# ModelTC/Dipoorlet

Measured on AMD Instinct MI355X. Metric: calibration images/sec (whole node) + achieved HBM GB/s, ResNet-50 ONNX N=1024, -A hist, higher is better.
Workload: dtype f32; 1 GPU; ResNet-50 ONNX activation set (T=123, 26598376 fp32 elems/img), -A hist --bins 2048, N=1024 per GPU in 32 batches of 32: range pass + histogram pass + percentile clip; device=AMD Radeon Graphics (gfx950:sramecc+:xnack-), hist_checksum_ok=True, world_size_seen_by_backend=1

## Files before the change

dipoorlet_amd/csrc/calib_kernels.hip:

```cpp
#include "common.hpp"

#pragma clang fp contract(off)

namespace {

struct MinMaxOp {
    float mn, mx;
    uint32_t nan;
    __device__ __forceinline__ void operator()(float x) {
        mn = fminf(mn, x);
        mx = fmaxf(mx, x);
        nan |= (x != x);
    }
};

__device__ __forceinline__ void minmax_commit(const MinMaxOp& op, uint32_t slot, float* s_mn, float* s_mx, uint32_t* s_nan,
                                              uint32_t* __restrict__ min_enc, uint32_t* __restrict__ max_enc,
                                              uint32_t* __restrict__ nan_flag) {
    float mn = wave_min(op.mn), mx = wave_max(op.mx);
    uint32_t nn = __any(op.nan) ? 1u : 0u;
    const int w = threadIdx.x / kWave;
    if ((threadIdx.x & (kWave - 1)) == 0) {
        s_mn[w] = mn;
        s_mx[w] = mx;
        s_nan[w] = nn;
    }
    __syncthreads();
    if (threadIdx.x == 0) {
#pragma unroll
        for (int j = 1; j < kBlock / kWave; ++j) {
            mn = fminf(mn, s_mn[j]);
            mx = fmaxf(mx, s_mx[j]);
            nn |= s_nan[j];
        }
        if (mn <= mx) {
            atomicMin(min_enc + slot, enc_f32(mn));
            atomicMax(max_enc + slot, enc_f32(mx));
        }
        if (nn) atomicOr(nan_flag + slot, 1u);
    }
    __syncthreads();
}

__global__ __launch_bounds__(kBlock) void k_minmax(const dpl_work_item* __restrict__ items,
                                                    const uint32_t* __restrict__ bb,
                                                    const float* const* __restrict__ segs,
                                                    uint32_t* __restrict__ min_enc, uint32_t* __restrict__ max_enc,
                                                    uint32_t* __restrict__ nan_flag) {
    __shared__ float s_mn[kBlock / kWave], s_mx[kBlock / kWave];
    __shared__ uint32_t s_nan[kBlock / kWave];
    uint32_t k0, k1;
    block_items(bb, k0, k1);
    for (uint32_t k = k0; k < k1; ++k) {
        const dpl_work_item it = items[k];
        MinMaxOp op{INFINITY, -INFINITY, 0u};
        stream_span(segs[it.seg] + it.offset, it.count, op);
        minmax_commit(op, it.slot, s_mn, s_mx, s_nan, min_enc, max_enc, nan_flag);
    }
}

__global__ void k_minmax_init(uint32_t* mn, uint32_t* mx, uint32_t* nan, int64_t n) {
    int64_t i = (int64_t)blockIdx.x * blockDim.x + threadIdx.x;
    if (i < n) {
        mn[i] = 0xFFFFFFFFu;
        mx[i] = 0u;
        nan[i] = 0u;
    }
}

__device__ __forceinline__ void minmax_decode(uint32_t mn, uint32_t mx, uint32_t nan, float& omn, float& omx) {
    const bool bad = nan != 0u || mn == 0xFFFFFFFFu;
    omn = bad ? NAN : dec_f32(mn);
    omx = bad ? NAN : dec_f32(mx);
}

__global__ void k_minmax_finalize(const uint32_t* mn, const uint32_t* mx, const uint32_t* nan, int64_t n,
                                  float* omn, float* omx) {
    int64_t i = (int64_t)blockIdx.x * blockDim.x + threadIdx.x;
    if (i < n) minmax_decode(mn[i], mx[i], nan[i], omn[i], omx[i]);
}

__global__ void k_minmax_encode(const float* mn, const float* mx, int64_t n, uint32_t* emn, uint32_t* emx,
                                uint32_t* nan) {
    int64_t i = (int64_t)blockIdx.x * blockDim.x + threadIdx.x;
    if (i < n) {
        const bool bad = (mn[i] != mn[i]) || (mx[i] != mx[i]);
        emn[i] = bad ? 0xFFFFFFFFu : enc_f32(mn[i]);
        emx[i] = bad ? 0u : enc_f32(mx[i]);
        nan[i] = bad ? 1u : 0u;
    }
}

__device__ __forceinline__ float hist_edge(int i, float step, float first) {
    return __fadd_rn(__fmul_rn((float)i, step), first);
}

template <bool kFast>
struct HistOp {
    uint32_t* lds;
    float first, last, step, inv, denom;
    int last_bin;
    float fbins;
    uint32_t nonzero;
    __device__ __forceinline__ void operator()(float x) {
        const float a = fabsf(x);
        const bool nz = (a != 0.0f);
        nonzero += nz;
        if (kFast) {
            if (nz && (a <= last)) {
                const int i = (int)__fmul_rn(a, inv);
                const uint32_t dec = (a < __fmul_rn((float)i, step)) ? 0xFFFFFFFCu : 0u;
                atomicAdd(reinterpret_cast<uint32_t*>(reinterpret_cast<char*>(lds) + (((uint32_t)i << 2) + dec)), 1u);
            }
            return;
        }
        int i;
        if (kFast) {
            i = (int)__fmul_rn(a, inv);
            i = i > last_bin ? last_bin : i;
            i -= (a < __fmul_rn((float)i, step)) ? 1 : 0;
        } else {
            i = (int)__fmul_rn(__fdiv_rn(__fsub_rn(a, first), denom), fbins);
            i = i > last_bin ? last_bin : i;
            i = i < 0 ? 0 : i;
            i -= (a < hist_edge(i, step, first)) ? 1 : 0;
            i += (i != last_bin && a >= hist_edge(i + 1, step, first)) ? 1 : 0;
        }
        if (nz && (a <= last)) atomicAdd(lds + i, 1u);
    }
};

template <bool kFast>
__device__ __forceinline__ void hist_op_init(HistOp<kFast>& op, const dpl_hist_range& r, int bins, uint32_t* lds) {
    op.lds = lds;
    op.first = r.first;
    op.last = r.last;
    op.step = r.step;
    op.inv = r.inv;
    op.denom = __fsub_rn(r.last, r.first);
    op.last_bin = bins - 1;
    op.fbins = (float)bins;
    op.nonzero = 0u;
}

template <class Count>
__device__ __forceinline__ void hist_flush(uint32_t nonzero, const dpl_work_item& it, const dpl_hist_range& r, int bins,
                                           Count* __restrict__ hist, uint32_t* lds, uint32_t* s_nz) {
    const uint32_t nzw = wave_sum(nonzero);
    if ((threadIdx.x & (kWave - 1)) == 0) s_nz[threadIdx.x / kWave] = nzw;
    __syncthreads();
    if (threadIdx.x == 0) {
        uint32_t nzb = 0;
        for (int k = 0; k < kBlock / kWave; ++k) nzb += s_nz[k];
        const uint32_t z = it.count - nzb;
        if (z) atomicAdd(lds + r.zero_bin, z);
        const uint32_t top = lds[bins];
        if (top) atomicAdd(lds + bins - 1, top);
    }
    __syncthreads();
    Count* __restrict__ out = hist + (uint64_t)it.slot * (uint64_t)bins;
    for (int b = threadIdx.x; b < bins; b += kBlock) {
        const uint32_t c = lds[b];
        if (c) {
            if constexpr (sizeof(Count) == 8)
                atomicAdd(reinterpret_cast<unsigned long long*>(out + b), (unsigned long long)c);
            else
                atomicAdd(out + b, c);
        }
    }
}

template <bool kFast>
__device__ __forceinline__ void hist_body(const dpl_work_item& it, const float* const* __restrict__ segs,
                                          const dpl_hist_range& r, int bins, uint64_t* __restrict__ hist,
                                          uint32_t* lds, uint32_t* s_nz) {
    HistOp<kFast> op;
    hist_op_init(op, r, bins, lds);
    stream_span(segs[it.seg] + it.offset, it.count, op);
    hist_flush(op.nonzero, it, r, bins, hist, lds, s_nz);
}

__global__ __launch_bounds__(kBlock) void k_abs_hist(const dpl_work_item* __restrict__ items,
                                                      const uint32_t* __restrict__ bb,
                                                      const float* const* __restrict__ segs,
                                                      const dpl_hist_range* __restrict__ ranges, int bins,
                                                      uint64_t* __restrict__ hist) {
    extern __shared__ __attribute__((aligned(16))) uint32_t lds[];
    uint32_t* s_nz = lds + bins + 1;
    uint32_t k0, k1;
    block_items(bb, k0, k1);
    for (uint32_t k = k0; k < k1; ++k) {
        const dpl_work_item it = items[k];
        const dpl_hist_range r = ranges[it.slot];
        if (r.status != 0u) continue;
        for (int b = threadIdx.x; b <= bins; b += kBlock) lds[b] = 0u;
        __syncthreads();
        if (r.exact_div)
            hist_body<false>(it, segs, r, bins, hist, lds, s_nz);
        else
            hist_body<true>(it, segs, r, bins, hist, lds, s_nz);
        __syncthreads();
    }
}

__device__ __forceinline__ float py_max(float a, float b) { return (b > a) ? b : a; }
__device__ __forceinline__ float py_min(float a, float b) { return (b < a) ? b : a; }

__device__ __forceinline__ dpl_hist_range hist_range_of(float gmin, float gmax, int bins) {
    dpl_hist_range r;
    const float dmax = py_max(gmax, -gmin);
    float first = 0.0f, last = dmax;
    r.dmax = dmax;
    r.status = 0u;
    if (!(fabsf(last) <= 3.402823466e+38f) || last < first) r.status = 1u;
    if (first == last) {
        first = -0.5f;
        last = 0.5f;
    }
    const float delta = __fsub_rn(last, first);
    const float fb = (float)bins;
    r.first = first;
    r.last = last;
    r.step = __fdiv_rn(delta, fb);
    r.inv = __fmul_rn(__fdiv_rn(fb, delta), 1.000001f);
    if (r.status == 0u) {
        const float e1 = hist_edge(1, r.step, first);
        const float el = hist_edge(bins - 1, r.step, first);
        const float el2 = hist_edge(bins - 2 > 0 ? bins - 2 : 0, r.step, first);
        if (!(r.step > 0.0f) || !(e1 > first) || !(last > el) || (bins > 2 && !(el > el2))) r.status = 2u;
    }
    r.exact_div = (first != 0.0f || !(fabsf(r.inv) <= 3.402823466e+38f) || r.step < 1.0e-30f) ? 1u : 0u;
    {
        const float a = 0.0f;
        float t = __fmul_rn(__fdiv_rn(__fsub_rn(a, first), delta), fb);
        int b = (int)t;
        b = b > bins - 1 ? bins - 1 : b;
        b = b < 0 ? 0 : b;
        if (a < hist_edge(b, r.step, first)) --b;
        if (b != bins - 1 && a >= hist_edge(b + 1, r.step, first)) ++b;
        r.zero_bin = (uint32_t)(b < 0 ? 0 : b);
    }
    return r;
}

__global__ void k_hist_prepare(const float* __restrict__ gmin, const float* __restrict__ gmax, int64_t n, int bins,
                               dpl_hist_range* __restrict__ out) {
    int64_t i = (int64_t)blockIdx.x * blockDim.x + threadIdx.x;
    if (i >= n) return;
    out[i] = hist_range_of(gmin[i], gmax[i], bins);
}

__host__ __device__ inline uint64_t spec_counts_offset(int64_t n_slots) {
    return (((uint64_t)n_slots * (sizeof(dpl_hist_range) + sizeof(uint32_t))) + 15ull) & ~15ull;
}

__global__ __launch_bounds__(kBlock) void k_hist_snapshot(const uint32_t* __restrict__ mn, const uint32_t* __restrict__ mx,
                                                           const uint32_t* __restrict__ nan, int64_t n, int bins,
                                                           dpl_hist_range* __restrict__ snap, uint32_t* __restrict__ flags,
                                                           uint32_t* __restrict__ counts) {
    const int64_t i = (int64_t)blockIdx.x * blockDim.x + threadIdx.x;
    const int64_t stride = (int64_t)gridDim.x * blockDim.x;
    if (i < n) {
        float gmin, gmax;
        minmax_decode(mn[i], mx[i], nan[i], gmin, gmax);
        snap[i] = hist_range_of(gmin, gmax, bins);
        flags[i] = 0u;
    }
    const int64_t total = n * (int64_t)bins;
    for (int64_t j = i; j < total; j += stride) counts[j] = 0u;
}

template <bool kFast>
struct MinMaxHistOp {
    MinMaxOp m;
    HistOp<kFast> h;
    __device__ __forceinline__ void operator()(float x) {
        m(x);
        h(x);
    }
};

template <bool kFast>
__device__ __forceinline__ void minmax_hist_body(const dpl_work_item& it, const float* const* __restrict__ segs,
                                                 const dpl_hist_range& r, int bins, uint32_t* __restrict__ counts,
                                                 uint32_t* lds, uint32_t* s_nz, MinMaxOp& m) {
    MinMaxHistOp<kFast> op;
    op.m = m;
    hist_op_init(op.h, r, bins, lds);
    stream_span(segs[it.seg] + it.offset, it.count, op);
    m = op.m;
    hist_flush(op.h.nonzero, it, r, bins, counts, lds, s_nz);
}

__global__ __launch_bounds__(kBlock) void k_minmax_hist(const dpl_work_item* __restrict__ items,
                                                         const uint32_t* __restrict__ bb,
                                                         const float* const* __restrict__ segs,
                                                         uint32_t* __restrict__ min_enc, uint32_t* __restrict__ max_enc,
                                                         uint32_t* __restrict__ nan_flag,
                                                         const dpl_hist_range* __restrict__ snap, int bins,
                                                         uint32_t* __restrict__ counts) {
    extern __shared__ __attribute__((aligned(16))) uint32_t lds_mh[];
    uint32_t* s_nz = lds_mh + bins + 1;
    float* s_mn = reinterpret_cast<float*>(s_nz + kBlock / kWave);
    float* s_mx = s_mn + kBlock / kWave;
    uint32_t* s_nan = reinterpret_cast<uint32_t*>(s_mx + kBlock / kWave);
    uint32_t k0, k1;
    block_items(bb, k0, k1);
    for (uint32_t k = k0; k < k1; ++k) {
        const dpl_work_item it = items[k];
        const dpl_hist_range r = snap[it.slot];
        MinMaxOp m{INFINITY, -INFINITY, 0u};
        if (r.status != 0u) {
            stream_span(segs[it.seg] + it.offset, it.count, m);
        } else {
            for (int b = threadIdx.x; b <= bins; b += kBlock) lds_mh[b] = 0u;
            __syncthreads();
            if (r.exact_div)
                minmax_hist_body<false>(it, segs, r, bins, counts, lds_mh, s_nz, m);
            else
                minmax_hist_body<true>(it, segs, r, bins, counts, lds_mh, s_nz, m);
        }
        minmax_commit(m, it.slot, s_mn, s_mx, s_nan, min_enc, max_enc, nan_flag);
    }
}

__global__ __launch_bounds__(kBlock) void k_hist_resolve(const dpl_hist_range* __restrict__ snap,
                                                          const dpl_hist_range* __restrict__ fin,
                                                          const uint32_t* __restrict__ counts, const uint64_t* __restrict__ elems,
                                                          int bins, uint64_t* __restrict__ hist, uint32_t* __restrict__ flags,
                                                          unsigned long long* __restrict__ stats) {
    const uint32_t t = blockIdx.x;
    const uint32_t* a = reinterpret_cast<const uint32_t*>(snap + t);
    const uint32_t* b = reinterpret_cast<const uint32_t*>(fin + t);
    bool same = true;
#pragma unroll
    for (int w = 0; w < (int)(sizeof(dpl_hist_range) / 4); ++w) same = same && (a[w] == b[w]);
    const uint32_t status = fin[t].status;
    const bool valid = same && status == 0u;
    if (threadIdx.x == 0) {
        flags[t] = valid ? 1u : (status != 0u ? 2u : 0u);
        if (stats) {
            const unsigned long long e = elems[t];
            atomicAdd(stats + 0, 1ull);
            atomicAdd(stats + 2, e);
            if (valid) {
                atomicAdd(stats + 1, 1ull);
                atomicAdd(stats + 3, e);
            }
        }
    }
    if (!valid) return;
    const uint32_t* __restrict__ row = counts + (uint64_t)t * (uint64_t)bins;
    uint64_t* __restrict__ out = hist + (uint64_t)t * (uint64_t)bins;
    for (int j = threadIdx.x; j < bins; j += kBlock) {
        const uint32_t c = row[j];
        if (c) out[j] += (uint64_t)c;
    }
}

__device__ __forceinline__ uint64_t shfl_up_u64(uint64_t v, int d) {
    const uint32_t lo = __shfl_up((uint32_t)v, d, kWave), hi = __shfl_up((uint32_t)(v >> 32), d, kWave);
    return ((uint64_t)hi << 32) | lo;
}

__device__ __forceinline__ void rest_prefix(const uint64_t* __restrict__ elems, const uint32_t* __restrict__ flags, int n_tensors,
                                            uint64_t* P, uint64_t* s_tot) {
    const int per = (n_tensors + kBlock - 1) / kBlock;
    const int t0 = (int)threadIdx.x * per;
    uint64_t mine = 0;
    for (int j = 0; j < per; ++j) {
        const int t = t0 + j;
        if (t < n_tensors && flags[t] == 0u) mine += elems[t];
    }
    uint64_t incl = mine;
    const int lane = threadIdx.x & (kWave - 1), wv = threadIdx.x / kWave;
#pragma unroll
    for (int o = 1; o < kWave; o <<= 1) {
        const uint64_t up = shfl_up_u64(incl, o);
        if (lane >= o) incl += up;
    }
    if (lane == kWave - 1) s_tot[wv] = incl;
    __syncthreads();
    uint64_t run = incl - mine;
    for (int w = 0; w < wv; ++w) run += s_tot[w];
    for (int j = 0; j < per; ++j) {
        const int t = t0 + j;
        if (t < n_tensors) {
            P[t] = run;
            if (flags[t] == 0u) run += elems[t];
        }
    }
    if (threadIdx.x == kBlock - 1) P[n_tensors] = run;
    __syncthreads();
}

__device__ __forceinline__ void rest_cut(const uint64_t* P, int n_tensors, uint64_t G, uint64_t b, uint64_t& cut, int& at) {
    const uint64_t total = P[n_tensors], q = total / G, rem = total % G;
    const uint64_t target = (b >= G) ? total : q * b + (rem * b) / G;
    if (target >= total) {
        cut = total;
        at = n_tensors;
        return;
    }
    int lo = 1, hi = n_tensors;
    while (lo < hi) {
        const int mid = (lo + hi) >> 1;
        if (P[mid] > target) hi = mid; else lo = mid + 1;
    }
    at = lo - 1;
    cut = P[lo - 1] + ((target - P[lo - 1]) & ~1023ull);
}

__global__ __launch_bounds__(kBlock) void k_abs_hist_rest(const uint64_t* __restrict__ elems, const uint32_t* __restrict__ flags,
                                                           int n_tensors, const float* const* __restrict__ segs,
                                                           const dpl_hist_range* __restrict__ ranges, int bins,
                                                           uint64_t* __restrict__ hist) {
    extern __shared__ __attribute__((aligned(16))) uint32_t lds_rest[];
    uint64_t* P = reinterpret_cast<uint64_t*>(lds_rest);
    uint64_t* s_tot = P + n_tensors + 1;
    uint32_t* lds = reinterpret_cast<uint32_t*>(s_tot + kBlock / kWave);
    uint32_t* s_nz = lds + bins + 1;
    rest_prefix(elems, flags, n_tensors, P, s_tot);
    if (P[n_tensors] == 0) return;
    uint64_t cut[2];
    int at[2];
    rest_cut(P, n_tensors, gridDim.x, blockIdx.x, cut[0], at[0]);
    rest_cut(P, n_tensors, gridDim.x, (uint64_t)blockIdx.x + 1, cut[1], at[1]);
    uint64_t pos = cut[0];
    const uint64_t end = cut[1];
    int t = at[0];
    while (pos < end) {
        while (P[t + 1] <= pos) ++t;
        const uint64_t stop = P[t + 1] < end ? P[t + 1] : end;
        dpl_work_item it;
        it.offset = pos - P[t];
        it.count = (uint32_t)(stop - pos);
        it.seg = (uint32_t)t;
        it.slot = (uint32_t)t;
        it.reserved = 0u;
        const dpl_hist_range r = ranges[t];
        for (int b = threadIdx.x; b <= bins; b += kBlock) lds[b] = 0u;
        __syncthreads();
        if (r.exact_div)
            hist_body<false>(it, segs, r, bins, hist, lds, s_nz);
        else
            hist_body<true>(it, segs, r, bins, hist, lds, s_nz);
        __syncthreads();
        pos = stop;
    }
}

__global__ __launch_bounds__(kBlock) void k_hist_spec_cuts(const uint64_t* __restrict__ elems, const uint32_t* __restrict__ flags,
                                                            int n_tensors, uint64_t* __restrict__ cuts) {
    extern __shared__ __attribute__((aligned(16))) uint32_t lds_cuts[];
    uint64_t* P = reinterpret_cast<uint64_t*>(lds_cuts);
    uint64_t* s_tot = P + n_tensors + 1;
    rest_prefix(elems, flags, n_tensors, P, s_tot);
    if (threadIdx.x != 0) return;
    uint64_t cut = 0;
    int at = 0;
    if (P[n_tensors] != 0) rest_cut(P, n_tensors, gridDim.x, blockIdx.x, cut, at);
    cuts[blockIdx.x] = cut;
    if (blockIdx.x + 1 == gridDim.x) cuts[gridDim.x] = P[n_tensors];
}

__device__ __forceinline__ void store_bin_clip(int found, float gmin, float gmax, int bins, float* __restrict__ clip) {
    float lo = gmin, hi = gmax;
    if (found >= 0) {
        const float dmax = py_max(-gmin, gmax);
        const float cv = __fmul_rn((float)found + 0.5f, __fdiv_rn(dmax, (float)bins));
        lo = py_max(-cv, gmin);
        hi = py_min(cv, gmax);
    }
    clip[0] = lo;
    clip[1] = hi;
}

__global__ __launch_bounds__(kWave) void k_hist_percentile(const uint64_t* __restrict__ hist,
                                                            const float* __restrict__ gmin_a,
                                                            const float* __restrict__ gmax_a, int bins,
                                                            double threshold, float* __restrict__ clip) {
    const int slot = blockIdx.x;
    const int lane = threadIdx.x;
    const uint64_t* h = hist + (uint64_t)slot * bins;
    unsigned long long tot = 0;
    for (int b = lane; b < bins; b += kWave) tot += h[b];
#pragma unroll
    for (int o = 32; o > 0; o >>= 1) tot += __shfl_xor(tot, o, kWave);
    const double total = (double)(long long)tot;
    const float gmin = gmin_a[slot], gmax = gmax_a[slot];
    double accum = 0.0;
    int found = -1;
    uint64_t raw_next = lane < bins ? h[lane] : 0ull;
    for (int base = 0; base < bins && found < 0; base += kWave) {
        const int b = base + lane;
        const double hv = (b < bins) ? (double)(float)(long long)raw_next / total : 0.0;
        raw_next = (b + kWave < bins) ? h[b + kWave] : 0ull;
        const int lim = (bins - base) < kWave ? (bins - base) : kWave;
        const int h_lo = __double2loint(hv), h_hi = __double2hiint(hv);
        uint64_t reached = 0;
        if (lim == kWave) {
#pragma unroll
            for (int j = 0; j < kWave; ++j) {
                accum += __hiloint2double(__builtin_amdgcn_readlane(h_hi, j), __builtin_amdgcn_readlane(h_lo, j));
                reached |= (accum >= threshold) ? (1ull << j) : 0ull;
            }
        } else {
            for (int j = 0; j < lim; ++j) {
                accum += __hiloint2double(__builtin_amdgcn_readlane(h_hi, j), __builtin_amdgcn_readlane(h_lo, j));
                reached |= (accum >= threshold) ? (1ull << j) : 0ull;
            }
        }
        if (reached) found = base + __builtin_ctzll(reached);
    }
    if (lane == 0) store_bin_clip(found, gmin, gmax, bins, clip + 2 * slot);
}

constexpr double kKlEps = 1e-4;

__device__ __forceinline__ uint32_t kl_live_below(const uint64_t* __restrict__ mask, const uint32_t* __restrict__ bcnt, uint32_t x) {
    const uint32_t k = x >> 6;
    return bcnt[k] + (uint32_t)__popcll(mask[k] & ((1ull << (x & 63u)) - 1ull));
}

__global__ __launch_bounds__(kBlock) void k_hist_kl(const uint64_t* __restrict__ hist, int bins, int levels, int n_chunks,
                                                     double* __restrict__ div) {
    extern __shared__ __attribute__((aligned(16))) uint64_t kl_lds[];
    const uint32_t nblk = ((uint32_t)bins + 63u) >> 6;
    uint64_t* cs = kl_lds;
    uint64_t* mask = cs + bins + 1;
    uint64_t* part = mask + nblk + 1;
    uint32_t* bcnt = reinterpret_cast<uint32_t*>(part + kBlock);
    const uint32_t tid = threadIdx.x, lane = tid & (kWave - 1), wave = tid / kWave;
    const uint32_t slot = blockIdx.x / (uint32_t)n_chunks, chunk = blockIdx.x % (uint32_t)n_chunks;
    const uint64_t* __restrict__ h = hist + (uint64_t)slot * (uint64_t)bins;
    double* __restrict__ out = div + (uint64_t)slot * ((uint64_t)bins + 1u);
    const uint32_t L = (uint32_t)levels, C = (uint32_t)n_chunks, nb = (uint32_t)bins;

    {
        const uint32_t per = (nb + kBlock - 1) / kBlock;
        const uint32_t b0 = tid * per < nb ? tid * per : nb, b1 = b0 + per < nb ? b0 + per : nb;
        uint64_t s = 0;
        for (uint32_t b = b0; b < b1; ++b) s += h[b];
        part[tid] = s;
        for (uint32_t k = wave; k < nblk; k += kBlock / kWave) {
            const uint32_t b = k * kWave + lane;
            const uint64_t m = __ballot(b < nb && h[b] != 0ull);
            if (lane == 0) mask[k] = m;
        }
        if (tid == 0) mask[nblk] = 0ull;
        __syncthreads();
        uint64_t off = 0;
        for (uint32_t j = 0; j < (uint32_t)kBlock; ++j) off += j < tid ? part[j] : 0ull;
        for (uint32_t b = b0; b < b1; ++b) {
            cs[b] = off;
            off += h[b];
        }
        if (tid == kBlock - 1) cs[nb] = off;
        for (uint32_t k = tid; k <= nblk; k += kBlock) {
            uint32_t a = 0;
            for (uint32_t j = 0; j < nblk; ++j) a += j < k ? (uint32_t)__popcll(mask[j]) : 0u;
            bcnt[k] = a;
        }
        __syncthreads();
    }
    for (uint32_t i = chunk + tid * C; i < L; i += kBlock * C) out[i] = INFINITY;

    const uint64_t N = cs[nb];
    const double dN = (double)(long long)N;
    const uint32_t first = L + (chunk + C - L % C) % C;
    for (uint32_t i = first + wave * C; i <= nb; i += (kBlock / kWave) * C) {
        const uint64_t csi = cs[i];
        const uint64_t outl = N - csi;
        const uint32_t s_last = (uint32_t)(((uint64_t)(L - 1u) * i) / L);
        const uint32_t woke = (csi == cs[i - 1] && outl != 0ull) ? 1u : 0u;
        const uint32_t n1p = kl_live_below(mask, bcnt, i) + woke;
        const uint32_t n1q = n1p - ((csi == cs[s_last] && outl != 0ull) ? 1u : 0u);
        double res = INFINITY;
        if (n1p != 0u && n1q != 0u) {
            const uint32_t zp = i - n1p, zq = i - n1q;
            const double e1p = kKlEps * (double)zp / (double)n1p;
            const double e1q = kKlEps * (double)zq / (double)n1q;
            if (e1p < 1.0 && e1q < 1.0) {
                const double Sp = dN - (double)n1p * e1p + (double)zp * kKlEps;
                const double Sq = (double)(long long)csi - (double)n1q * e1q + (double)zq * kKlEps;
                double acc = 0.0;
                for (uint32_t b = lane; b < i; b += kWave) {
                    uint64_t pb = cs[b + 1] - cs[b];
                    if (b == i - 1u) pb += outl;
                    if (pb != 0ull) {
                        const uint32_t g = ((b + 1u) * L - 1u) / i;
                        const uint32_t s0 = (g * i) / L, s1 = ((g + 1u) * i) / L;
                        const uint64_t G = cs[s1] - cs[s0];
                        double qs = kKlEps;
                        if (G != 0ull) {
                            const uint32_t live = kl_live_below(mask, bcnt, s1) - kl_live_below(mask, bcnt, s0) + (s1 == i ? woke : 0u);
                            qs = (double)(long long)G / (double)live - e1q;
                        }
                        const double P = ((double)(long long)pb - e1p) / Sp, Q = qs / Sq;
                        acc += P * log(P / Q);
                    }
                }
                acc = wave_sum(acc);
                const double Pz = kKlEps / Sp, Qz = kKlEps / Sq;
                res = acc + (double)zp * (Pz * log(Pz / Qz));
            }
        }
        if (lane == 0) out[i] = res;
    }
}

__global__ __launch_bounds__(kWave) void k_hist_kl_pick(const double* __restrict__ div, const float* __restrict__ gmin_a,
                                                         const float* __restrict__ gmax_a, int bins, int32_t* __restrict__ best,
                                                         float* __restrict__ clip) {
    const int slot = blockIdx.x;
    const int lane = threadIdx.x;
    const double* __restrict__ d = div + (uint64_t)slot * ((uint64_t)bins + 1u);
    double bv = INFINITY;
    int bi = -1;
    for (int i = lane; i <= bins; i += kWave) {
        const double v = d[i];
        if (v < bv) {
            bv = v;
            bi = i;
        }
    }
#pragma unroll
    for (int o = 32; o > 0; o >>= 1) {
        const double ov = __shfl_xor(bv, o, kWave);
        const int oi = __shfl_xor(bi, o, kWave);
        if (ov < bv || (ov == bv && oi >= 0 && (bi < 0 || oi < bi))) {
            bv = ov;
            bi = oi;
        }
    }
    if (lane == 0) {
        best[slot] = bi;
        store_bin_clip(bi >= 0 ? bi - 1 : -1, gmin_a[slot], gmax_a[slot], bins, clip + 2 * slot);
    }
}

constexpr int kGridUniform = DPL_GRID_UNIFORM, kGridE4M3 = DPL_GRID_E4M3;

template <int GRID>
__global__ __launch_bounds__(kBlock) void k_hist_qmse(const uint64_t* __restrict__ hist, int bins, int first, int top, int n_chunks,
                                                       double* __restrict__ err) {
    extern __shared__ __attribute__((aligned(16))) double qm_lds[];
    double* hd = qm_lds;
    uint64_t* part = reinterpret_cast<uint64_t*>(hd + bins);
    const uint32_t tid = threadIdx.x, lane = tid & (kWave - 1), wave = tid / kWave;
    const uint32_t slot = blockIdx.x / (uint32_t)n_chunks, chunk = blockIdx.x % (uint32_t)n_chunks;
    const uint64_t* __restrict__ h = hist + (uint64_t)slot * (uint64_t)bins;
    double* __restrict__ out = err + (uint64_t)slot * ((uint64_t)bins + 1u);
    const uint32_t F = (uint32_t)first, C = (uint32_t)n_chunks, nb = (uint32_t)bins;

    uint64_t s = 0;
    for (uint32_t b = tid; b < nb; b += kBlock) {
        const uint64_t v = h[b];
        s += v;
        hd[b] = (double)(long long)v;
    }
#pragma unroll
    for (int o = 32; o > 0; o >>= 1) s += __shfl_xor(s, o, kWave);
    if (lane == 0) part[wave] = s;
    __syncthreads();
    uint64_t N = 0;
#pragma unroll
    for (int w = 0; w < kBlock / kWave; ++w) N += part[w];

    for (uint32_t i = chunk + tid * C; i < F; i += kBlock * C) out[i] = INFINITY;

    constexpr double unit = GRID == kGridE4M3 ? 512.0 : 1.0;
    const double dtop = GRID == kGridE4M3 ? 448.0 : (double)top;
    const double atop = unit * dtop;
    const double norm = (double)(long long)N * (4.0 * atop * atop);
    for (uint32_t i = F + chunk + wave * C; i <= nb; i += (kBlock / kWave) * C) {
        const double t = (double)(2u * i - 1u);
        const double rt = 1.0 / (unit * t);
        double acc = 0.0;
        if (N != 0ull) {
            for (uint32_t b = lane; b < nb; b += kWave) {
                const double hb = hd[b];
                if (hb != 0.0) {
                    const double a = (double)(2u * b + 1u) * atop;
                    const double v = fmin(a * rt, dtop);
                    double q;
                    if (GRID == kGridE4M3) {
                        int e = (int)((__double_as_longlong(v) >> 52) & 0x7FF) - 1023;
                        e = e < -6 ? -6 : e;
                        const double istep = __longlong_as_double((long long)(1023 + 3 - e) << 52);
                        const double step512 = __longlong_as_double((long long)(1023 + 9 - 3 + e) << 52);
                        q = rint(v * istep) * step512;
                    } else {
                        q = rint(v);
                    }
                    const double dt = a - q * t;
                    acc += hb * (dt * dt);
                }
            }
            acc = wave_sum(acc);
        }
        if (lane == 0) out[i] = N != 0ull ? acc / norm : INFINITY;
    }
}

__global__ __launch_bounds__(kBlock) void k_rowwise_minmax(const float* __restrict__ w, int64_t cols,
                                                            float* __restrict__ omn, float* __restrict__ omx) {
    __shared__ float s_mn[kBlock / kWave], s_mx[kBlock / kWave];
    __shared__ uint32_t s_nan[kBlock / kWave];
    const float* p = w + (int64_t)blockIdx.x * cols;
    MinMaxOp op{INFINITY, -INFINITY, 0u};
    stream_span(p, (uint32_t)cols, op);
    float mn = wave_min(op.mn), mx = wave_max(op.mx);
    uint32_t nn = __any(op.nan) ? 1u : 0u;
    const int wv = threadIdx.x / kWave;
    if ((threadIdx.x & (kWave - 1)) == 0) {
        s_mn[wv] = mn;
        s_mx[wv] = mx;
        s_nan[wv] = nn;
    }
    __syncthreads();
    if (threadIdx.x == 0) {
        for (int k = 1; k < kBlock / kWave; ++k) {
            mn = fminf(mn, s_mn[k]);
            mx = fmaxf(mx, s_mx[k]);
// ... 330 lines not shown
                    DPL_CEAT(PA, QA);
                    if (!(i + (kU - 1) * kBlock < nvec)) {
                        DPL_CEAT(PB, QB);
                        break;
                    }
                    DPL_CLOAD(PA, QA, i);
                    i += kStride;
                    DPL_CEAT(PB, QB);
                }
            }
#undef DPL_CLOAD
#undef DPL_CEAT
            for (; i < nvec; i += kBlock) eat1(__builtin_nontemporal_load(av + i), __builtin_nontemporal_load(bv + i));
            done = nvec << 2;
        }
        for (uint32_t i = done + threadIdx.x; i < n; i += kBlock) {
            const float p = a[i], q = b[i];
            ab += (double)p * q;
            aa += (double)p * p;
            bbs += (double)q * q;
        }
        ab = wave_sum(ab);
        aa = wave_sum(aa);
        bbs = wave_sum(bbs);
        const int w = threadIdx.x / kWave;
        if ((threadIdx.x & (kWave - 1)) == 0) {
            s_r[0][w] = ab;
            s_r[1][w] = aa;
            s_r[2][w] = bbs;
        }
        __syncthreads();
        if (threadIdx.x < 3) {
            double v = 0.0;
            for (int j = 0; j < kBlock / kWave; ++j) v += s_r[threadIdx.x][j];
            atomicAdd(acc + 3 * (uint64_t)it.slot + threadIdx.x, v);
        }
        __syncthreads();
    }
}

template <int FMT>
int fake_quant_launch(const char* who, int32_t pre, const float* d_x, const float* d_x2, float* d_y, int64_t n, const float* d_scale,
                      const int32_t* d_zp, int64_t n_channels, int64_t inner, int32_t qlo, int32_t qhi, dpl_stream_t s) {
    auto bad = [who](const char* what) {
        char m[192];
        snprintf(m, sizeof(m), "%s: %s", who, what);
        return fail_msg(m);
    };
    if (pre != DPL_FQ_PRE_NONE && pre != DPL_FQ_PRE_RELU && pre != DPL_FQ_PRE_ADD_RELU)
        return bad("pre must be DPL_FQ_PRE_NONE, _RELU or _ADD_RELU");
    if (n <= 0) return 0;
    if (pre == DPL_FQ_PRE_ADD_RELU && d_x2 == nullptr) return bad("DPL_FQ_PRE_ADD_RELU needs d_x2");
    if (n_channels < 1 || inner < 1 || n_channels > 0xFFFFFFFFll || inner > 0xFFFFFFFFll)
        return bad("n_channels and inner must be in [1, 2^32)");
    constexpr int64_t kFqChunk = 3072;
    int64_t chunk = kFqChunk;
    if ((n + chunk - 1) / chunk > 0x40000000ll) chunk = ((n + 0x3FFFFFFFll) / 0x40000000ll + 1023) / 1024 * 1024;
    if (chunk > 0xFFFFFC00ll) chunk = 0xFFFFFC00ll;
    const int64_t blocks = (n + chunk - 1) / chunk;
    if (blocks > 0x7FFFFFFFll) return bad("tensor too large");
#define DPL_FQ_LAUNCH(PRE)                                                                                                    \
    hipLaunchKernelGGL((k_fake_quant<PRE, FMT>), dim3((unsigned)blocks), dim3(kBlock), 0, (hipStream_t)s, d_x, d_x2, d_y, (uint64_t)n,   \
                       (uint64_t)chunk, d_scale, d_zp, (uint32_t)n_channels, (uint32_t)inner, (float)qlo, (float)qhi)
    if (pre == DPL_FQ_PRE_ADD_RELU) DPL_FQ_LAUNCH(kFqPreAddRelu);
    else if (pre == DPL_FQ_PRE_RELU) DPL_FQ_LAUNCH(kFqPreRelu);
    else DPL_FQ_LAUNCH(kFqPreNone);
#undef DPL_FQ_LAUNCH
    DPL_LAUNCH_CHECK("k_fake_quant");
    return 0;
}

}

extern "C" {

int dpl_abi_version(void) { return DPL_ABI_VERSION; }
const char* dpl_last_error(void) { return g_err; }

int dpl_device_info(char* name, int name_cap, int* compute_units, uint64_t* hbm_bytes) {
    int dev = 0;
    hipError_t e = hipGetDevice(&dev);
    if (e != hipSuccess) return fail("hipGetDevice", e);
    hipDeviceProp_t p;
    e = hipGetDeviceProperties(&p, dev);
    if (e != hipSuccess) return fail("hipGetDeviceProperties", e);
    if (name && name_cap > 0) snprintf(name, name_cap, "%s (%s)", p.name, p.gcnArchName);
    if (compute_units) *compute_units = p.multiProcessorCount;
    if (hbm_bytes) *hbm_bytes = (uint64_t)p.totalGlobalMem;
    if (strncmp(p.gcnArchName, "gfx950", 6) != 0) return fail_msg("current HIP device is not gfx950");
    return 0;
}

int dpl_stream_priority_range(int* least, int* greatest) {
    int lo = 0, hi = 0;
    hipError_t e = hipDeviceGetStreamPriorityRange(&lo, &hi);
    if (e != hipSuccess) return fail("hipDeviceGetStreamPriorityRange", e);
    if (least) *least = lo;
    if (greatest) *greatest = hi;
    return 0;
}

int dpl_stream_create(int priority, dpl_stream_t* out) {
    if (!out) return fail_msg("dpl_stream_create: null out");
    int lo = 0, hi = 0;
    hipError_t e = hipDeviceGetStreamPriorityRange(&lo, &hi);
    if (e != hipSuccess) return fail("hipDeviceGetStreamPriorityRange", e);
    if (priority > lo) priority = lo;
    if (priority < hi) priority = hi;
    hipStream_t s = nullptr;
    e = hipStreamCreateWithPriority(&s, hipStreamNonBlocking, priority);
    if (e != hipSuccess) return fail("hipStreamCreateWithPriority", e);
    *out = (dpl_stream_t)s;
    return 0;
}

int dpl_stream_destroy(dpl_stream_t s) {
    if (!s) return 0;
    hipError_t e = hipStreamDestroy((hipStream_t)s);
    return e == hipSuccess ? 0 : fail("hipStreamDestroy", e);
}

int64_t dpl_build_work_items(const dpl_span* spans, int64_t n_spans, uint64_t chunk_elems, dpl_work_item* out,
                             int64_t cap) {
    if (!spans || n_spans < 0 || chunk_elems == 0 || (chunk_elems % 1024) != 0 || chunk_elems > 0xFFFFFC00ull)
        return fail_msg("dpl_build_work_items: chunk_elems must be a non-zero multiple of 1024 below 2^32");
    int64_t n = 0;
    for (int64_t i = 0; i < n_spans; ++i) {
        uint64_t off = spans[i].offset, left = spans[i].count;
        while (left) {
            const uint64_t c = left < chunk_elems ? left : chunk_elems;
            if (out && n < cap) {
                out[n].offset = off;
                out[n].count = (uint32_t)c;
                out[n].seg = spans[i].seg;
                out[n].slot = spans[i].slot;
                out[n].reserved = 0;
            }
            ++n;
            off += c;
            left -= c;
        }
    }
    return n;
}

int dpl_minmax_init(uint32_t* d_min_enc, uint32_t* d_max_enc, uint32_t* d_nan, int64_t n_slots, dpl_stream_t s) {
    if (n_slots <= 0) return 0;
    hipLaunchKernelGGL(k_minmax_init, dim3(grid_for(n_slots, 256)), dim3(256), 0, (hipStream_t)s, d_min_enc,
                       d_max_enc, d_nan, n_slots);
    DPL_LAUNCH_CHECK("k_minmax_init");
    return 0;
}

int64_t dpl_build_balanced_items(const dpl_span* spans, int64_t n_spans, int64_t n_blocks, dpl_work_item* out,
                                 int64_t cap, uint32_t* block_begin) {
    if (!spans || n_spans < 0 || n_blocks < 1) return fail_msg("dpl_build_balanced_items: bad arguments");
    unsigned __int128 total = 0;
    for (int64_t i = 0; i < n_spans; ++i) total += spans[i].count;
    int64_t n = 0;
    int64_t si = 0;
    uint64_t lo = 0;
    unsigned __int128 g = 0;
    for (int64_t b = 0; b < n_blocks; ++b) {
        if (block_begin) block_begin[b] = (uint32_t)n;
        const unsigned __int128 target = (b + 1 == n_blocks) ? total : (total * (unsigned __int128)(b + 1)) / (unsigned __int128)n_blocks;
        while (si < n_spans && g < target) {
            const uint64_t remaining = spans[si].count - lo;
            if (remaining == 0) {
                ++si;
                lo = 0;
                continue;
            }
            const unsigned __int128 want = target - g;
            uint64_t take;
            bool span_done;
            if (want >= remaining) {
                take = remaining;
                span_done = true;
            } else {
                take = ((uint64_t)want / 1024u) * 1024u;
                span_done = false;
                if (take == 0) break;
            }
            uint64_t off = spans[si].offset + lo, left = take;
            while (left) {
                const uint64_t c = left < 0xFFFFFC00ull ? left : 0xFFFFFC00ull;
                if (out && n < cap) {
                    out[n].offset = off;
                    out[n].count = (uint32_t)c;
                    out[n].seg = spans[si].seg;
                    out[n].slot = spans[si].slot;
                    out[n].reserved = 0;
                }
                ++n;
                off += c;
                left -= c;
            }
            g += take;
            lo += take;
            if (span_done) {
                ++si;
                lo = 0;
            } else {
                break;
            }
        }
    }
    if (block_begin) block_begin[n_blocks] = (uint32_t)n;
    return n;
}

int dpl_minmax_accumulate(const dpl_work_item* d_items, int64_t n_items, const uint32_t* d_block_begin,
                          int64_t n_blocks, const float* const* d_seg_ptrs, uint32_t* d_min_enc,
                          uint32_t* d_max_enc, uint32_t* d_nan, dpl_stream_t s) {
    if (n_items <= 0) return 0;
    if (int e = check_blocks("dpl_minmax_accumulate", n_items, d_block_begin, n_blocks)) return e;
    hipLaunchKernelGGL(k_minmax, dim3((unsigned)n_blocks), dim3(kBlock), 0, (hipStream_t)s, d_items, d_block_begin,
                       d_seg_ptrs, d_min_enc, d_max_enc, d_nan);
    DPL_LAUNCH_CHECK("k_minmax");
    return 0;
}

int dpl_minmax_finalize(const uint32_t* d_min_enc, const uint32_t* d_max_enc, const uint32_t* d_nan,
                        int64_t n_slots, float* d_min, float* d_max, dpl_stream_t s) {
    if (n_slots <= 0) return 0;
    hipLaunchKernelGGL(k_minmax_finalize, dim3(grid_for(n_slots, 256)), dim3(256), 0, (hipStream_t)s, d_min_enc,
                       d_max_enc, d_nan, n_slots, d_min, d_max);
    DPL_LAUNCH_CHECK("k_minmax_finalize");
    return 0;
}

int dpl_minmax_encode(const float* d_min, const float* d_max, int64_t n_slots, uint32_t* d_min_enc,
                      uint32_t* d_max_enc, uint32_t* d_nan, dpl_stream_t s) {
    if (n_slots <= 0) return 0;
    hipLaunchKernelGGL(k_minmax_encode, dim3(grid_for(n_slots, 256)), dim3(256), 0, (hipStream_t)s, d_min, d_max,
                       n_slots, d_min_enc, d_max_enc, d_nan);
    DPL_LAUNCH_CHECK("k_minmax_encode");
    return 0;
}

int dpl_hist_prepare(const float* d_min, const float* d_max, int64_t n_slots, int bins, dpl_hist_range* d_ranges,
                     dpl_stream_t s) {
    if (bins < 1 || bins > DPL_MAX_BINS) return fail_msg("dpl_hist_prepare: bins must be in [1, 16384]");
    if (n_slots <= 0) return 0;
    hipLaunchKernelGGL(k_hist_prepare, dim3(grid_for(n_slots, 64)), dim3(64), 0, (hipStream_t)s, d_min, d_max,
                       n_slots, bins, d_ranges);
    DPL_LAUNCH_CHECK("k_hist_prepare");
    return 0;
}

int dpl_abs_hist_accumulate(const dpl_work_item* d_items, int64_t n_items, const uint32_t* d_block_begin,
                            int64_t n_blocks, const float* const* d_seg_ptrs, const dpl_hist_range* d_ranges,
                            int bins, uint64_t* d_hist, dpl_stream_t s) {
    if (bins < 1 || bins > DPL_MAX_BINS) return fail_msg("dpl_abs_hist_accumulate: bins must be in [1, 16384]");
    if (n_items <= 0) return 0;
    if (int e = check_blocks("dpl_abs_hist_accumulate", n_items, d_block_begin, n_blocks)) return e;
    hipLaunchKernelGGL(k_abs_hist, dim3((unsigned)n_blocks), dim3(kBlock),
                       ((size_t)bins + 1 + kBlock / kWave) * sizeof(uint32_t), (hipStream_t)s, d_items, d_block_begin,
                       d_seg_ptrs, d_ranges, bins, d_hist);
    DPL_LAUNCH_CHECK("k_abs_hist");
    return 0;
}

uint64_t dpl_hist_spec_entry_bytes(int64_t n_slots, int bins) {
    if (n_slots < 0 || bins < 1 || bins > DPL_MAX_BINS) return 0;
    return spec_counts_offset(n_slots) + (uint64_t)n_slots * (uint64_t)bins * sizeof(uint32_t);
}

int dpl_minmax_hist_accumulate(const dpl_work_item* d_items, int64_t n_items, const uint32_t* d_block_begin,
                               int64_t n_blocks, const float* const* d_seg_ptrs, uint32_t* d_min_enc, uint32_t* d_max_enc,
                               uint32_t* d_nan, int64_t n_slots, int bins, void* d_entry, dpl_stream_t s) {
    if (bins < 1 || bins > DPL_MAX_BINS) return fail_msg("dpl_minmax_hist_accumulate: bins must be in [1, 16384]");
    if (!d_entry || ((uintptr_t)d_entry & 15u)) return fail_msg("dpl_minmax_hist_accumulate: d_entry must be 16-byte aligned");
    if (n_slots <= 0 || n_slots > 0x7FFFFFFFll) return fail_msg("dpl_minmax_hist_accumulate: n_slots out of range");
    if (n_items <= 0) return 0;
    if (int e = check_blocks("dpl_minmax_hist_accumulate", n_items, d_block_begin, n_blocks)) return e;
    dpl_hist_range* snap = (dpl_hist_range*)d_entry;
    uint32_t* flags = (uint32_t*)(snap + n_slots);
    uint32_t* counts = (uint32_t*)((char*)d_entry + spec_counts_offset(n_slots));
    int64_t zb = grid_for(n_slots * (int64_t)bins, kBlock * 8);
    if (zb < grid_for(n_slots, kBlock)) zb = grid_for(n_slots, kBlock);
    if (zb > 1024) zb = 1024;
    hipLaunchKernelGGL(k_hist_snapshot, dim3((unsigned)zb), dim3(kBlock), 0, (hipStream_t)s, d_min_enc, d_max_enc, d_nan,
                       n_slots, bins, snap, flags, counts);
    DPL_LAUNCH_CHECK("k_hist_snapshot");
    hipLaunchKernelGGL(k_minmax_hist, dim3((unsigned)n_blocks), dim3(kBlock),
                       ((size_t)bins + 1 + 4 * (kBlock / kWave)) * sizeof(uint32_t), (hipStream_t)s, d_items, d_block_begin,
                       d_seg_ptrs, d_min_enc, d_max_enc, d_nan, snap, bins, counts);
    DPL_LAUNCH_CHECK("k_minmax_hist");
    return 0;
}

int dpl_hist_spec_accumulate(void* d_entry, const uint64_t* d_elems, int64_t n_slots, int64_t n_blocks,
                             const float* const* d_seg_ptrs, const dpl_hist_range* d_ranges, int bins, uint64_t* d_hist,
                             uint64_t* d_stats, dpl_stream_t s) {
    if (bins < 1 || bins > DPL_MAX_BINS) return fail_msg("dpl_hist_spec_accumulate: bins must be in [1, 16384]");
    if (!d_entry || ((uintptr_t)d_entry & 15u)) return fail_msg("dpl_hist_spec_accumulate: d_entry must be 16-byte aligned");
    if (n_slots <= 0 || n_slots > DPL_HIST_SPEC_MAX_TENSORS)
        return fail_msg("dpl_hist_spec_accumulate: n_slots must be in [1, DPL_HIST_SPEC_MAX_TENSORS]");
    if (n_blocks <= 0 || n_blocks > 0x7FFFFFFFll) return fail_msg("dpl_hist_spec_accumulate: n_blocks out of range");
    dpl_hist_range* snap = (dpl_hist_range*)d_entry;
    uint32_t* flags = (uint32_t*)(snap + n_slots);
    const uint32_t* counts = (const uint32_t*)((char*)d_entry + spec_counts_offset(n_slots));
    hipLaunchKernelGGL(k_hist_resolve, dim3((unsigned)n_slots), dim3(kBlock), 0, (hipStream_t)s, snap, d_ranges, counts, d_elems,
                       bins, d_hist, flags, (unsigned long long*)d_stats);
    DPL_LAUNCH_CHECK("k_hist_resolve");
    const size_t lds = ((size_t)n_slots + 1 + kBlock / kWave) * sizeof(uint64_t) + ((size_t)bins + 1 + kBlock / kWave) * sizeof(uint32_t);
    hipLaunchKernelGGL(k_abs_hist_rest, dim3((unsigned)n_blocks), dim3(kBlock), lds, (hipStream_t)s, d_elems, flags, (int)n_slots,
                       d_seg_ptrs, d_ranges, bins, d_hist);
    DPL_LAUNCH_CHECK("k_abs_hist_rest");
    return 0;
}

int dpl_hist_spec_cuts(const void* d_entry, const uint64_t* d_elems, int64_t n_slots, int64_t n_blocks, uint64_t* d_cuts,
                       dpl_stream_t s) {
    if (!d_entry || !d_cuts) return fail_msg("dpl_hist_spec_cuts: null argument");
    if (n_slots <= 0 || n_slots > DPL_HIST_SPEC_MAX_TENSORS)
        return fail_msg("dpl_hist_spec_cuts: n_slots must be in [1, DPL_HIST_SPEC_MAX_TENSORS]");
    if (n_blocks <= 0 || n_blocks > 0x7FFFFFFFll) return fail_msg("dpl_hist_spec_cuts: n_blocks out of range");
    const uint32_t* flags = (const uint32_t*)((const dpl_hist_range*)d_entry + n_slots);
    hipLaunchKernelGGL(k_hist_spec_cuts, dim3((unsigned)n_blocks), dim3(kBlock),
                       ((size_t)n_slots + 1 + kBlock / kWave) * sizeof(uint64_t), (hipStream_t)s, d_elems, flags, (int)n_slots, d_cuts);
    DPL_LAUNCH_CHECK("k_hist_spec_cuts");
    return 0;
}

int dpl_hist_percentile(const uint64_t* d_hist, const float* d_min, const float* d_max, int64_t n_slots, int bins,
                        double threshold, float* d_clip, dpl_stream_t s) {
    if (n_slots <= 0) return 0;
    hipLaunchKernelGGL(k_hist_percentile, dim3((unsigned)n_slots), dim3(kWave), 0, (hipStream_t)s, d_hist, d_min,
                       d_max, bins, threshold, d_clip);
    DPL_LAUNCH_CHECK("k_hist_percentile");
    return 0;
}

int dpl_hist_kl(const uint64_t* d_hist, const float* d_min, const float* d_max, int64_t n_slots, int bins, int levels,
                double* d_div, int32_t* d_best, float* d_clip, dpl_stream_t s) {
    if (bins < 1 || bins > DPL_MAX_BINS) return fail_msg("dpl_hist_kl: bins must be in [1, 16384]");
    if (levels < 2 || levels > bins) return fail_msg("dpl_hist_kl: levels must be in [2, bins]");
    if (n_slots <= 0) return 0;
    const int64_t n_cand = (int64_t)bins - levels + 1;
    int64_t chunks = (1024 + n_slots - 1) / n_slots;
    if (chunks > n_cand / 8) chunks = n_cand / 8;
    if (chunks < 1) chunks = 1;
    if (n_slots * chunks > 0x7FFFFFFFll) return fail_msg("dpl_hist_kl: too many slots");
    const size_t nblk = ((size_t)bins + 63) / 64;
    const size_t lds = ((size_t)bins + 1 + nblk + 1 + kBlock) * sizeof(uint64_t) + (nblk + 1) * sizeof(uint32_t);
    hipLaunchKernelGGL(k_hist_kl, dim3((unsigned)(n_slots * chunks)), dim3(kBlock), lds, (hipStream_t)s, d_hist, bins, levels,
                       (int)chunks, d_div);
    DPL_LAUNCH_CHECK("k_hist_kl");
    hipLaunchKernelGGL(k_hist_kl_pick, dim3((unsigned)n_slots), dim3(kWave), 0, (hipStream_t)s, d_div, d_min, d_max, bins,
                       d_best, d_clip);
    DPL_LAUNCH_CHECK("k_hist_kl_pick");
    return 0;
}

int dpl_hist_qmse(const uint64_t* d_hist, const float* d_min, const float* d_max, int64_t n_slots, int bins, int first, int grid,
                  int top, double* d_err, int32_t* d_best, float* d_clip, dpl_stream_t s) {
    if (bins < 1 || bins > DPL_MAX_BINS) return fail_msg("dpl_hist_qmse: bins must be in [1, 16384]");
    if (first < 1 || first > bins) return fail_msg("dpl_hist_qmse: first must be in [1, bins]");
    if (grid != DPL_GRID_UNIFORM && grid != DPL_GRID_E4M3) return fail_msg("dpl_hist_qmse: grid must be DPL_GRID_UNIFORM or DPL_GRID_E4M3");
    if (grid == DPL_GRID_UNIFORM && (top < 1 || top > 32767)) return fail_msg("dpl_hist_qmse: top must be in [1, 32767] on the uniform grid");
    if (grid == DPL_GRID_E4M3 && top != 0) return fail_msg("dpl_hist_qmse: top must be 0 on the E4M3 grid (its largest value is 448)");
    if (n_slots <= 0) return 0;
    const int64_t n_cand = (int64_t)bins - first + 1;
    int64_t chunks = (1024 + n_slots - 1) / n_slots;
    if (chunks > n_cand / 8) chunks = n_cand / 8;
    if (chunks < 1) chunks = 1;
    if (n_slots * chunks > 0x7FFFFFFFll) return fail_msg("dpl_hist_qmse: too many slots");
    const size_t lds = (size_t)bins * sizeof(double) + (kBlock / kWave) * sizeof(uint64_t);
    const dim3 wgs((unsigned)(n_slots * chunks));
    if (grid == DPL_GRID_E4M3)
        hipLaunchKernelGGL(k_hist_qmse<kGridE4M3>, wgs, dim3(kBlock), lds, (hipStream_t)s, d_hist, bins, first, top, (int)chunks, d_err);
    else
        hipLaunchKernelGGL(k_hist_qmse<kGridUniform>, wgs, dim3(kBlock), lds, (hipStream_t)s, d_hist, bins, first, top, (int)chunks, d_err);
    DPL_LAUNCH_CHECK("k_hist_qmse");
    hipLaunchKernelGGL(k_hist_kl_pick, dim3((unsigned)n_slots), dim3(kWave), 0, (hipStream_t)s, d_err, d_min, d_max, bins,
                       d_best, d_clip);
    DPL_LAUNCH_CHECK("k_hist_kl_pick");
    return 0;
}

int dpl_rowwise_minmax(const float* d_w, int64_t rows, int64_t cols, float* d_min, float* d_max, dpl_stream_t s) {
    if (rows <= 0) return 0;
    if (cols <= 0 || cols > 0xFFFFFFFFll) return fail_msg("dpl_rowwise_minmax: cols out of range");
    hipLaunchKernelGGL(k_rowwise_minmax, dim3((unsigned)rows), dim3(kBlock), 0, (hipStream_t)s, d_w, cols, d_min,
                       d_max);
    DPL_LAUNCH_CHECK("k_rowwise_minmax");
    return 0;
}

int dpl_fake_quant(const float* d_x, float* d_y, int64_t n, const float* d_scale, const int32_t* d_zp,
                   int64_t n_channels, int64_t inner, int32_t qlo, int32_t qhi, dpl_stream_t s) {
    return dpl_fake_quant_pre(DPL_FQ_PRE_NONE, d_x, nullptr, d_y, n, d_scale, d_zp, n_channels, inner, qlo, qhi, s);
}

int dpl_fake_quant_pre(int32_t pre, const float* d_x, const float* d_x2, float* d_y, int64_t n, const float* d_scale,
                       const int32_t* d_zp, int64_t n_channels, int64_t inner, int32_t qlo, int32_t qhi, dpl_stream_t s) {
    return fake_quant_launch<kFqFmtInt>("dpl_fake_quant_pre", pre, d_x, d_x2, d_y, n, d_scale, d_zp, n_channels, inner, qlo, qhi, s);
}

int dpl_fake_quant_fp8(int32_t pre, const float* d_x, const float* d_x2, float* d_y, int64_t n, const float* d_scale,
                       int64_t n_channels, int64_t inner, dpl_stream_t s) {
    return fake_quant_launch<kFqFmtE4M3>("dpl_fake_quant_fp8", pre, d_x, d_x2, d_y, n, d_scale, nullptr, n_channels, inner, 0, 0, s);
}

int dpl_fake_quant_items(const dpl_work_item* d_items, int64_t n_items, const uint32_t* d_block_begin, int64_t n_blocks,
                         const float* const* d_seg_x, float* const* d_seg_y, const dpl_fake_quant_params* d_params, dpl_stream_t s) {
    if (n_items <= 0) return 0;
    if (int e = check_blocks("dpl_fake_quant_items", n_items, d_block_begin, n_blocks)) return e;
    hipLaunchKernelGGL(k_fake_quant_items<kFqFmtInt>, dim3((unsigned)n_blocks), dim3(kBlock), 0, (hipStream_t)s, d_items, d_block_begin,
                       d_seg_x, d_seg_y, d_params);
    DPL_LAUNCH_CHECK("k_fake_quant_items");
    return 0;
}

int dpl_fake_quant_fp8_items(const dpl_work_item* d_items, int64_t n_items, const uint32_t* d_block_begin, int64_t n_blocks,
                             const float* const* d_seg_x, float* const* d_seg_y, const dpl_fake_quant_params* d_params, dpl_stream_t s) {
    if (n_items <= 0) return 0;
    if (int e = check_blocks("dpl_fake_quant_fp8_items", n_items, d_block_begin, n_blocks)) return e;
    hipLaunchKernelGGL(k_fake_quant_items<kFqFmtE4M3>, dim3((unsigned)n_blocks), dim3(kBlock), 0, (hipStream_t)s, d_items, d_block_begin,
                       d_seg_x, d_seg_y, d_params);
    DPL_LAUNCH_CHECK("k_fake_quant_fp8_items");
    return 0;
}

int dpl_cos_accumulate(const float* d_a, const float* d_b, int64_t n, double* d_acc, int64_t slot, dpl_stream_t s) {
    if (n <= 0) return 0;
    if (((uintptr_t)d_a | (uintptr_t)d_b) & 15u) return fail_msg("dpl_cos_accumulate: buffers must be 16-B aligned");
    int64_t blocks = (n / 4 + kBlock * 8 - 1) / (kBlock * 8);
    if (blocks < 1) blocks = 1;
    if (blocks > 2048) blocks = 2048;
    hipLaunchKernelGGL(k_cos_acc, dim3((unsigned)blocks), dim3(kBlock), 0, (hipStream_t)s, d_a, d_b, n,
                       d_acc + 3 * slot);
    DPL_LAUNCH_CHECK("k_cos_acc");
    return 0;
}

int dpl_channel_diff_sum(const float* d_a, const float* d_b, int64_t outer, int64_t n_channels, int64_t inner,
                         double* d_acc, dpl_stream_t s) {
    if (outer <= 0 || n_channels <= 0 || inner <= 0) return 0;
    if (n_channels > 0xFFFFFFFFll || inner > 0xFFFFFFFFll) return fail_msg("dpl_channel_diff_sum: extent out of range");
    const uint64_t rows = (uint64_t)outer * (uint64_t)n_channels;
    const int vec_ok = ((inner & 3) == 0) && ((((uintptr_t)d_a | (uintptr_t)d_b) & 15u) == 0);
    uint64_t work = inner == 1 ? (uint64_t)(n_channels + kWave - 1) / kWave : rows;
    uint64_t blocks = (work + kBlock / kWave - 1) / (kBlock / kWave);
    if (blocks < 1) blocks = 1;
    if (blocks > 256 * 16) blocks = 256 * 16;
    hipLaunchKernelGGL(k_channel_diff_sum, dim3((unsigned)blocks), dim3(kBlock), 0, (hipStream_t)s, d_a, d_b, rows,
                       (uint32_t)n_channels, (uint32_t)inner, vec_ok, d_acc);
    DPL_LAUNCH_CHECK("k_channel_diff_sum");
    return 0;
}

int dpl_cos_items_accumulate(const dpl_work_item* d_items, int64_t n_items, const uint32_t* d_block_begin,
                             int64_t n_blocks, const float* const* d_seg_a, const float* const* d_seg_b,
                             double* d_acc, dpl_stream_t s) {
    if (n_items <= 0) return 0;
    if (int e = check_blocks("dpl_cos_items_accumulate", n_items, d_block_begin, n_blocks)) return e;
    hipLaunchKernelGGL(k_cos_items, dim3((unsigned)n_blocks), dim3(kBlock), 0, (hipStream_t)s, d_items,
                       d_block_begin, d_seg_a, d_seg_b, d_acc);
    DPL_LAUNCH_CHECK("k_cos_items");
    return 0;
}

}
```

Measured before the change: 56410 images/s.

## Fuse speculative histogram resolve into rest kernel and vectorize count merges

Merges the per-tensor resolve kernel into the rest-histogram kernel. Every block recomputes the snapshot-vs-final verdict into LDS byte flags, and blocks grid-stride over tensors to fold valid speculative counts into the 64-bit histogram. Row adds are batched and vectorized with uint4/ulonglong2 loads, and the count-zeroing in the snapshot kernel now uses uint4 stores. This saves one launch and the dependency between the two kernels, at the cost of redundant verdict computation in each block and unconditional writes to hist rows.

```diff
diff --git a/dipoorlet_amd/csrc/calib_kernels.hip b/dipoorlet_amd/csrc/calib_kernels.hip
--- a/dipoorlet_amd/csrc/calib_kernels.hip
+++ b/dipoorlet_amd/csrc/calib_kernels.hip
@@ -266,8 +266,10 @@
         snap[i] = hist_range_of(gmin, gmax, bins);
         flags[i] = 0u;
     }
-    const int64_t total = n * (int64_t)bins;
-    for (int64_t j = i; j < total; j += stride) counts[j] = 0u;
+    const int64_t total = n * (int64_t)bins, quads = total >> 2;
+    uint4* c4 = reinterpret_cast<uint4*>(counts);
+    for (int64_t q = i; q < quads; q += stride) c4[q] = make_uint4(0u, 0u, 0u, 0u);
+    for (int64_t j = (quads << 2) + i; j < total; j += stride) counts[j] = 0u;
 }
 
 template <bool kFast>
@@ -324,37 +326,67 @@
     }
 }
 
-__global__ __launch_bounds__(kBlock) void k_hist_resolve(const dpl_hist_range* __restrict__ snap,
-                                                          const dpl_hist_range* __restrict__ fin,
-                                                          const uint32_t* __restrict__ counts, const uint64_t* __restrict__ elems,
-                                                          int bins, uint64_t* __restrict__ hist, uint32_t* __restrict__ flags,
-                                                          unsigned long long* __restrict__ stats) {
-    const uint32_t t = blockIdx.x;
+__device__ __forceinline__ uint32_t spec_verdict(const dpl_hist_range* __restrict__ snap, const dpl_hist_range* __restrict__ fin,
+                                                 int t) {
     const uint32_t* a = reinterpret_cast<const uint32_t*>(snap + t);
     const uint32_t* b = reinterpret_cast<const uint32_t*>(fin + t);
-    bool same = true;
+    uint32_t diff = 0u;
 #pragma unroll
-    for (int w = 0; w < (int)(sizeof(dpl_hist_range) / 4); ++w) same = same && (a[w] == b[w]);
+    for (int w = 0; w < (int)(sizeof(dpl_hist_range) / 4); ++w) diff |= a[w] ^ b[w];
     const uint32_t status = fin[t].status;
-    const bool valid = same && status == 0u;
-    if (threadIdx.x == 0) {
-        flags[t] = valid ? 1u : (status != 0u ? 2u : 0u);
-        if (stats) {
-            const unsigned long long e = elems[t];
-            atomicAdd(stats + 0, 1ull);
-            atomicAdd(stats + 2, e);
-            if (valid) {
-                atomicAdd(stats + 1, 1ull);
-                atomicAdd(stats + 3, e);
-            }
-        }
-    }
-    if (!valid) return;
-    const uint32_t* __restrict__ row = counts + (uint64_t)t * (uint64_t)bins;
-    uint64_t* __restrict__ out = hist + (uint64_t)t * (uint64_t)bins;
-    for (int j = threadIdx.x; j < bins; j += kBlock) {
-        const uint32_t c = row[j];
-        if (c) out[j] += (uint64_t)c;
+    return (diff == 0u && status == 0u) ? 1u : (status != 0u ? 2u : 0u);
+}
+
+constexpr int kRowBatch = 4;
+
+__device__ __forceinline__ void spec_row_add(const uint32_t* __restrict__ row, uint64_t* __restrict__ out, int bins, bool vec) {
+    if (vec) {
+        const uint4* __restrict__ r4 = reinterpret_cast<const uint4*>(row);
+        ulonglong2* __restrict__ o2 = reinterpret_cast<ulonglong2*>(out);
+        const int groups = bins >> 2;
+        for (int g0 = threadIdx.x; g0 < groups; g0 += kRowBatch * kBlock) {
+            uint4 c[kRowBatch];
+            ulonglong2 lo[kRowBatch], hi[kRowBatch];
+#pragma unroll
+            for (int u = 0; u < kRowBatch; ++u) {
+                const int g = g0 + u * kBlock;
+                if (g < groups) {
+                    c[u] = r4[g];
+                    lo[u] = o2[2 * g];
+                    hi[u] = o2[2 * g + 1];
+                }
+            }
+#pragma unroll
+            for (int u = 0; u < kRowBatch; ++u) {
+                const int g = g0 + u * kBlock;
+                if (g < groups) {
+                    lo[u].x += c[u].x;
+                    lo[u].y += c[u].y;
+                    hi[u].x += c[u].z;
+                    hi[u].y += c[u].w;
+                    o2[2 * g] = lo[u];
+                    o2[2 * g + 1] = hi[u];
+                }
+            }
+        }
+        return;
+    }
+    for (int j0 = threadIdx.x; j0 < bins; j0 += kRowBatch * kBlock) {
+        uint32_t c[kRowBatch];
+        uint64_t h[kRowBatch];
+#pragma unroll
+        for (int u = 0; u < kRowBatch; ++u) {
+            const int j = j0 + u * kBlock;
+            if (j < bins) {
+                c[u] = row[j];
+                h[u] = out[j];
+            }
+        }
+#pragma unroll
+        for (int u = 0; u < kRowBatch; ++u) {
+            const int j = j0 + u * kBlock;
+            if (j < bins) out[j] = h[u] + (uint64_t)c[u];
+        }
     }
 }
 
@@ -363,7 +395,8 @@
     return ((uint64_t)hi << 32) | lo;
 }
 
-__device__ __forceinline__ void rest_prefix(const uint64_t* __restrict__ elems, const uint32_t* __restrict__ flags, int n_tensors,
+template <class Flag>
+__device__ __forceinline__ void rest_prefix(const uint64_t* __restrict__ elems, const Flag* flags, int n_tensors,
                                             uint64_t* P, uint64_t* s_tot) {
     const int per = (n_tensors + kBlock - 1) / kBlock;
     const int t0 = (int)threadIdx.x * per;
@@ -411,16 +444,38 @@
     cut = P[lo - 1] + ((target - P[lo - 1]) & ~1023ull);
 }
 
-__global__ __launch_bounds__(kBlock) void k_abs_hist_rest(const uint64_t* __restrict__ elems, const uint32_t* __restrict__ flags,
-                                                           int n_tensors, const float* const* __restrict__ segs,
-                                                           const dpl_hist_range* __restrict__ ranges, int bins,
-                                                           uint64_t* __restrict__ hist) {
-    extern __shared__ __attribute__((aligned(16))) uint32_t lds_rest[];
-    uint64_t* P = reinterpret_cast<uint64_t*>(lds_rest);
+__global__ __launch_bounds__(kBlock) void k_hist_spec(const dpl_hist_range* __restrict__ snap,
+                                                       const dpl_hist_range* __restrict__ ranges,
+                                                       const uint32_t* __restrict__ counts, const uint64_t* __restrict__ elems,
+                                                       int n_tensors, const float* const* __restrict__ segs, int bins,
+                                                       uint64_t* __restrict__ hist, uint32_t* __restrict__ flags,
+                                                       unsigned long long* __restrict__ stats) {
+    extern __shared__ __attribute__((aligned(16))) uint32_t lds_spec[];
+    uint64_t* P = reinterpret_cast<uint64_t*>(lds_spec);
     uint64_t* s_tot = P + n_tensors + 1;
     uint32_t* lds = reinterpret_cast<uint32_t*>(s_tot + kBlock / kWave);
     uint32_t* s_nz = lds + bins + 1;
-    rest_prefix(elems, flags, n_tensors, P, s_tot);
+    uint8_t* s_flag = reinterpret_cast<uint8_t*>(s_nz + kBlock / kWave);
+    for (int t = threadIdx.x; t < n_tensors; t += kBlock) s_flag[t] = (uint8_t)spec_verdict(snap, ranges, t);
+    __syncthreads();
+    const bool vec = (bins & 3) == 0 && ((reinterpret_cast<uintptr_t>(counts) | reinterpret_cast<uintptr_t>(hist)) & 15u) == 0;
+    for (uint64_t t = blockIdx.x; t < (uint64_t)n_tensors; t += gridDim.x) {
+        const uint32_t f = s_flag[t];
+        if (threadIdx.x == 0) {
+            flags[t] = f;
+            if (stats) {
+                const unsigned long long e = elems[t];
+                atomicAdd(stats + 0, 1ull);
+                atomicAdd(stats + 2, e);
+                if (f == 1u) {
+                    atomicAdd(stats + 1, 1ull);
+                    atomicAdd(stats + 3, e);
+                }
+            }
+        }
+        if (f == 1u) spec_row_add(counts + t * (uint64_t)bins, hist + t * (uint64_t)bins, bins, vec);
+    }
+    rest_prefix(elems, s_flag, n_tensors, P, s_tot);
     if (P[n_tensors] == 0) return;
     uint64_t cut[2];
     int at[2];
@@ -1357,13 +1412,11 @@
     dpl_hist_range* snap = (dpl_hist_range*)d_entry;
     uint32_t* flags = (uint32_t*)(snap + n_slots);
     const uint32_t* counts = (const uint32_t*)((char*)d_entry + spec_counts_offset(n_slots));
-    hipLaunchKernelGGL(k_hist_resolve, dim3((unsigned)n_slots), dim3(kBlock), 0, (hipStream_t)s, snap, d_ranges, counts, d_elems,
-                       bins, d_hist, flags, (unsigned long long*)d_stats);
-    DPL_LAUNCH_CHECK("k_hist_resolve");
-    const size_t lds = ((size_t)n_slots + 1 + kBlock / kWave) * sizeof(uint64_t) + ((size_t)bins + 1 + kBlock / kWave) * sizeof(uint32_t);
-    hipLaunchKernelGGL(k_abs_hist_rest, dim3((unsigned)n_blocks), dim3(kBlock), lds, (hipStream_t)s, d_elems, flags, (int)n_slots,
-                       d_seg_ptrs, d_ranges, bins, d_hist);
-    DPL_LAUNCH_CHECK("k_abs_hist_rest");
+    const size_t lds = ((size_t)n_slots + 1 + kBlock / kWave) * sizeof(uint64_t) + ((size_t)bins + 1 + kBlock / kWave) * sizeof(uint32_t) +
+                       (((size_t)n_slots + 3) & ~(size_t)3);
+    hipLaunchKernelGGL(k_hist_spec, dim3((unsigned)n_blocks), dim3(kBlock), lds, (hipStream_t)s, snap, d_ranges, counts, d_elems,
+                       (int)n_slots, d_seg_ptrs, bins, d_hist, flags, (unsigned long long*)d_stats);
+    DPL_LAUNCH_CHECK("k_hist_spec");
     return 0;
 }
 
```

Measured after the change: 56860 images/s, median of 6. Within noise of the previous version (+0.8%).
